# hbaatz/nerf-tex

Measured on AMD Instinct MI355X. Metric: ray-samples/sec (MLP+composite) at 800x800x64, higher is better.
Workload: dtype f32; 1 GPU; carpet 800x800x64: 640000 all-hit rays x 64 samples per GPU (BASELINE configs[1]), ParamNerf n_parameters=[1, 6], seeded glorot weights, inputs resident in HBM, fused PE+MLP+composite; rays_per_gpu=640000, hit_rays_total=640000, samples_per_ray=64

## Files before the change

nerf_tex_amd/csrc/ntx_backend_chain.hip:

```cpp
#include <algorithm>
#include <cstdio>
#include <cstdlib>
#include "ntx_trainer.h"
#include "ntx_train_device.h"
#include "ntx_encode.h"
namespace ntx_train {
enum { PACK_HIDDEN = 0, PACK_LINEAR = 1, PACK_AUX_ROW = 2, PACK_AUX_RGB = 3, PACK_COPY = 4 };
struct PackSeg {
    const float *src; long long sk, sc;
    int mode;
    int K, ncols, nt;
    float *dst; long long first, count;
};
struct PackArgs { const PackSeg *seg; int n_seg; long long total; };
__global__ void pack_kernel(PackArgs a) {
    const long long e = (long long)blockIdx.x * blockDim.x + threadIdx.x;
    if (e >= a.total) return;
    int lo = 0, hi = a.n_seg - 1;
    while (lo < hi) { const int mid = (lo + hi + 1) >> 1; if (a.seg[mid].first <= e) lo = mid; else hi = mid - 1; }
    const PackSeg &p = a.seg[lo];
    const long long o = e - p.first;
    float v = 0.0f;
    if (p.mode == PACK_COPY) v = p.src[o];
    else if (p.mode == PACK_AUX_ROW) {
        const int h = (int)(o >> 7) & 1, V = (int)(o & 127), k = hidden_row(V, h);
        v = k < p.K ? p.src[k * p.sk] : 0.0f;
    } else if (p.mode == PACK_AUX_RGB) {
        const int c = (int)(o >> 7), h = (int)(o >> 6) & 1, V = (int)(o & 63);
        v = p.src[hidden_row(V, h) * 3 + c];
    } else {
        const int c = (int)(o & 3), lane = (int)((o >> 2) & 63);
        const long long rec = o >> 8;
        const int G = p.nt / 4, g = (int)(rec % G), s = (int)(rec / G);
        const int f = lane & 31, kh = lane >> 5;
        const int k = p.mode == PACK_HIDDEN ? hidden_row(s, kh) : 2 * s + kh, col = 32 * (4 * g + c) + f;
        if (k < p.K && col < p.ncols) v = p.src[k * p.sk + col * p.sc];
    }
    p.dst[o] = v;
}

struct EncodeArgs {
    StepRays r;
    float *posO; int ptiles;
    float *dirO; int dtiles;
    float *dists;
};
template <bool IPE>
__global__ __launch_bounds__(64) void encode_kernel(EncodeArgs args) {
    const StepRays &a = args.r;
    const int lane = threadIdx.x, n = lane & 31, h = lane >> 5, blk = blockIdx.x, part = blockIdx.y;
    const long long m = (long long)blk * 32 + n;
    const bool valid = m < a.M();
    const int ray = valid ? (int)(m / a.S) : 0, s = valid ? (int)(m - (long long)ray * a.S) : 0;
// ... 154 lines not shown
            }); });
        }
    }
}

}
namespace {
using namespace ntx_train;
struct ChainBackend : Backend {
    ntx_trainer *t = nullptr;
    int ptiles = 0, dtiles = 0, PS = 0, DS = 0, fwd_variant = 0;
    TLayer trunk[8], feature, c1, c2, rgb, alpha;
    float *wfwd = nullptr, *wdx = nullptr, *aux = nullptr; size_t fwd_floats = 0, dx_floats = 0;
    PackSeg *pack_seg = nullptr; int n_pack = 0; long long pack_total = 0;
    float *posO = nullptr, *dirO = nullptr;
    float *act = nullptr; long long act_stride = 0;
    unsigned int *bits = nullptr; long long bits_stride = 0;
    float *dirrow = nullptr;
    float *gout = nullptr; long long gout_stride = 0;
    DwJob *jobs = nullptr; int n_jobs = 0; long long total_cost = 0;
    std::vector<DwJob> jobs_host; std::vector<int> reduce_job;
    float *dw_partial = nullptr; ReduceBatch reduce{};
    float *G_pos = nullptr, *G_dir = nullptr; int ld_pos = 0, ld_dir = 0;
    float *ray_pg = nullptr;
    float *act_at(int i) const { return act + (size_t)i * act_stride; }
    float *gout_at(int i) const { return gout + (size_t)i * gout_stride; }
    bool samples_on = false;
    static int blocks_of(long long rows) { return (int)((rows + 31) / 32); }
    unsigned chain_grid(long long rows) const { return (unsigned)std::min<long long>(t->cus, (blocks_of(rows) + 3) / 4); }
    unsigned feat_grid(long long rows) const { return (unsigned)std::min<long long>(2 * (long long)t->cus, (blocks_of(rows) + 3) / 4); }
// ... 42 lines not shown
    };
    auto seg = [&](const float *src, long long sk, long long sc, int mode, int K, int ncols, int nt, int stream, int nsteps) {
        PackSeg s{}; s.src = src; s.sk = sk; s.sc = sc; s.mode = mode; s.K = K; s.ncols = ncols; s.nt = nt;
        const int ring = stream == DX ? DX_RING : RING;
        const long long recs = ((long long)nsteps * (nt / 4) + ring - 1) / ring * ring;
        push(s, stream, floats[stream], recs * 256); floats[stream] += (size_t)recs * 256;
    };
    const float *W = t->w;
    auto fwd_hidden = [&](const TLayer &l, int row0, int nt) { seg(W + l.w + (size_t)row0 * l.out, l.out, 1, PACK_HIDDEN, 256, l.out, nt, FWD, 128); };
    auto fwd_linear = [&](const TLayer &l, int K, int nsteps) { seg(W + l.w, l.out, 1, PACK_LINEAR, K, l.out, 8, FWD, nsteps); };
    fwd_linear(trunk[0], Kp, PS);
    for (int i = 1; i < 8; ++i) {
        if (i == 5) { fwd_linear(trunk[5], Kp, PS); fwd_hidden(trunk[5], Kp, 8); }
        else fwd_hidden(trunk[i], 0, 8);
    }
    fwd_hidden(feature, 0, 8);
    fwd_linear(c1, Kd, DS); fwd_hidden(c1, Kd, 8);
    fwd_hidden(c2, 0, 4);
    const size_t n_fwd_segs = segs.size();
    auto dx_hidden = [&](const TLayer &l, int row0, int K, int nsteps) { seg(W + l.w + (size_t)row0 * l.out, 1, l.out, PACK_HIDDEN, K, 256, 8, DX, nsteps); };
    seg(W + rgb.w, 1, 3, PACK_LINEAR, 3, 128, 4, DX, 2);
    dx_hidden(c2, 0, 128, 64);
    dx_hidden(c1, Kd, 256, 128);
    dx_hidden(feature, 0, 256, 128);
    seg(W + alpha.w, 1, 1, PACK_LINEAR, 1, 256, 8, DX, 1);
    for (int i = 7; i >= 1; --i) dx_hidden(trunk[i], i == 5 ? Kp : 0, 256, 128);
    auto tail = [&](size_t of, int stream) { const long long count = (long long)(stream == DX ? DX_RING : RING) * 256; push(segs[of], stream, floats[stream], count); floats[stream] += (size_t)count; };
    tail(0, FWD); tail(n_fwd_segs, DX);
    auto aux_seg = [&](const float *src, int mode, int K, long long count, size_t at) { PackSeg s{}; s.src = src; s.sk = 1; s.mode = mode; s.K = K; push(s, AUX, at, count); };
    for (int i = 0; i < 8; ++i) aux_seg(W + trunk[i].b, PACK_AUX_ROW, 256, 256, AUX_BIAS + (size_t)i * 256);
    aux_seg(W + feature.b, PACK_AUX_ROW, 256, 256, AUX_BIAS + 8 * 256); aux_seg(W + c1.b, PACK_AUX_ROW, 256, 256, AUX_BIAS + 9 * 256);
    aux_seg(W + c2.b, PACK_AUX_ROW, 128, 256, AUX_BIAS + 10 * 256);
    aux_seg(W + alpha.w, PACK_AUX_ROW, 256, 256, AUX_ALPHA_W); aux_seg(W + alpha.b, PACK_COPY, 1, 1, AUX_ALPHA_B);
    aux_seg(W + rgb.w, PACK_AUX_RGB, 128, 384, AUX_RGB_W); aux_seg(W + rgb.b, PACK_COPY, 3, 3, AUX_RGB_B);
    pack_total = first; n_pack = (int)segs.size(); fwd_floats = floats[FWD]; dx_floats = floats[DX];
    t->mem.alloc(&wfwd, fwd_floats); t->mem.alloc(&wdx, dx_floats); t->mem.alloc(&aux, AUX_FLOATS, true);
    float *const base[3] = {wfwd, wdx, aux};
    for (size_t i = 0; i < segs.size(); ++i) segs[i].dst = (float *)((char *)base[base_of[i]] + (uintptr_t)segs[i].dst);
    t->mem.upload(&pack_seg, segs, "segment");
}

void ChainBackend::build_dw_jobs() {
    const int Kp = t->Kp, Kd = t->Kd;
    std::vector<DwJob> &jobs = jobs_host;
    struct RJ { int job; long long at, count, pair; size_t out; };
    std::vector<RJ> rjobs;
    auto new_job = [&]() { DwJob j{}; for (DwWave &w : j.w) w.shape = -1; jobs.push_back(j); return (int)jobs.size() - 1; };
    auto matrix = [&](int j, int K, int N, size_t g_kernel, long long g_bias, long long *at_bias) {
        const long long at = jobs[j].slot_floats;
        jobs[j].slot_floats += (long long)K * N;
        rjobs.push_back(RJ{j, at, (long long)K * N, 0, g_kernel});
        *at_bias = -1;
        if (g_bias >= 0) { *at_bias = jobs[j].slot_floats; jobs[j].slot_floats += 2 * N; rjobs.push_back(RJ{j, *at_bias, N, N, (size_t)g_bias}); }
        return at;
    };
    auto wave = [&](int j, int w, int shape, const float *A, int rtA, int a0, const float *B, int rtB, int b0, long long at, int K, int N, int c_lo, long long at_bias) {
        DwWave &d = jobs[j].w[w];
        d.A = A; d.rtA = rtA; d.a0 = a0; d.B = B; d.rtB = rtB; d.b0 = b0; d.shape = shape; d.out = at; d.ldc = N; d.row0 = a0 * 32; d.rows_valid = K;
        d.col0 = b0 * 32; d.c_lo = c_lo; d.c_hi = c_lo + N; d.bias_out = a0 == 0 ? at_bias : -1;
        const int cost = shape == 0 ? 256 : shape == 1 ? 198 : 68;
        if (cost > jobs[j].cost) jobs[j].cost = cost;
    };
    auto layer_job = [&](const float *X, const float *dY, size_t g_kernel, size_t g_bias) {
        const int j = new_job(); long long ab; const long long at = matrix(j, 256, 256, g_kernel, (long long)g_bias, &ab);
        for (int w = 0; w < 4; ++w) wave(j, w, 0, X, 8, 4 * (w >> 1), dY, 8, 4 * (w & 1), at, 256, 256, 0, ab);
    };
    for (int i = 7; i >= 1; --i) layer_job(act_at(i - 1), gout_at(10 - i), trunk[i].w + (size_t)(i == 5 ? Kp : 0) * 256, trunk[i].b);
    layer_job(act_at(7), gout_at(2), feature.w, feature.b);
    layer_job(act_at(8), gout_at(1), c1.w + (size_t)Kd * 256, c1.b);
    {
        const int j = new_job(); long long ab0, ab5;
        const long long at0 = matrix(j, Kp, 256, trunk[0].w, (long long)trunk[0].b, &ab0), at5 = matrix(j, Kp, 256, trunk[5].w, -1, &ab5);
        for (int w = 0; w < 2; ++w) { wave(j, w, 1, posO, ptiles, 0, gout_at(10), 8, 4 * w, at0, Kp, 256, 0, ab0); wave(j, 2 + w, 1, posO, ptiles, 0, gout_at(5), 8, 4 * w, at5, Kp, 256, 0, ab5); }
    }
    {
        const int j = new_job(); long long abd, ab2;
        const long long atd = matrix(j, Kd, 256, c1.w, -1, &abd), at2 = matrix(j, 256, 128, c2.w, (long long)c2.b, &ab2);
        for (int w = 0; w < 2; ++w) { wave(j, w, 1, dirO, dtiles, 0, gout_at(1), 8, 4 * w, atd, Kd, 256, 0, abd); wave(j, 2 + w, 0, act_at(9), 8, 4 * w, gout_at(0), 4, 0, at2, 256, 128, 0, ab2); }
    }
    {
        const int j = new_job(); long long abr, aba;
        const long long atr = matrix(j, 128, 3, rgb.w, (long long)rgb.b, &abr), ata = matrix(j, 256, 1, alpha.w, (long long)alpha.b, &aba);
        wave(j, 0, 2, act_at(10), 4, 0, t->dhead, 1, 0, atr, 128, 3, 0, abr);
        for (int w = 0; w < 2; ++w) wave(j, 1 + w, 2, act_at(7), 8, 4 * w, t->dhead, 1, 0, ata, 256, 1, 3, aba);
    }
    n_jobs = (int)jobs.size();
    size_t partial_floats = 0;
    for (DwJob &j : jobs) total_cost += j.cost;
    for (DwJob &j : jobs) {
        const long long slots = ((long long)j.cost * t->cus + total_cost - 1) / total_cost + 2;
        j.first_float = (long long)partial_floats; partial_floats += (size_t)(slots * j.slot_floats);
    }
    t->mem.alloc(&dw_partial, partial_floats);
    t->mem.upload(&this->jobs, jobs, "job");
    if (t->mem.rc == NTX_OK && (int)rjobs.size() > MAX_REDUCE_BATCH) t->mem.rc = ntx_set_error(NTX_E_INVALID, "trainer: too many weight gradients for one launch");
    long long rfirst = 0;
    for (size_t i = 0; i < rjobs.size() && t->mem.rc == NTX_OK; ++i) {
        ReduceJob &r = reduce.job[reduce.n++];
        const DwJob &j = jobs[rjobs[i].job];
        r.partial = dw_partial + j.first_float + rjobs[i].at; r.n_split = 0; r.stride = j.slot_floats; r.count = rjobs[i].count; r.pair = rjobs[i].pair;
        r.out = t->grad + rjobs[i].out; r.first = rfirst;
        rfirst += (rjobs[i].count + 255) / 256 * 256;
        reduce_job.push_back(rjobs[i].job);
    }
}

void ChainBackend::launch_pack(hipStream_t st) {
    const PackArgs pa{pack_seg, n_pack, pack_total};
    hipLaunchKernelGGL(pack_kernel, dim3((unsigned)((pack_total + 255) / 256)), dim3(256), 0, st, pa);
}
FwdArgs ChainBackend::fwd_args(long long M) const {
    FwdArgs f{}; f.stream = wfwd; f.stream_bytes = (uint32_t)(fwd_floats * sizeof(float)); f.aux = aux; f.M = M;
    f.ptiles = ptiles; f.dtiles = dtiles; f.pos = posO; f.dir = dirO;
    f.act = act; f.act_stride = act_stride; f.bits = bits; f.bits_stride = bits_stride;
    f.sigma = t->sigma; f.raw_rgb = t->raw_rgb;
    return f;
}
int ChainBackend::forward(const StepRays &r, hipStream_t st) {
    launch_pack(st);
    EncodeArgs e{}; e.r = r; e.posO = posO; e.ptiles = ptiles; e.dirO = dirO; e.dtiles = dtiles; e.dists = t->dists;
    if (t->ipe) hipLaunchKernelGGL(encode_kernel<true>, dim3((unsigned)r.n_blocks(), 2), dim3(64), 0, st, e);
    else hipLaunchKernelGGL(encode_kernel<false>, dim3((unsigned)r.n_blocks(), 2), dim3(64), 0, st, e);
    FwdArgs f = fwd_args(r.M());
    const bool hoist = (t->ipe || r.blur_idx < 0 || r.blur_idx < r.n_geo) && r.S % 32 == 0 && getenv("NERFTEX_TRAIN_NO_DIR_HOIST") == nullptr;
    if (hoist) {
        DirRowArgs dr{}; dr.r = r; dr.Kd = t->Kd; dr.w = t->w + c1.w; dr.bias = t->w + c1.b; dr.rows = dirrow; dr.splice = t->ipe ? r.blur_idx : -1;
        hipLaunchKernelGGL(dirrow_kernel, dim3((unsigned)r.n_rays), dim3(256), 0, st, dr);
    }
    f.dirrow = dirrow; f.n_rays = (int)r.n_rays; f.S = r.S;
    launch_fwd_chain(fwd_variant, hoist, st, chain_grid(r.M()), f);
    return NTX_OK;
}
int ChainBackend::forward_samples(const StepSamples &s, hipStream_t st) {
    if (int rc = takes_samples()) return rc;
    const long long M = s.n_live;
    if (M == 0) return NTX_OK;
    launch_pack(st);
    EncodeSamplesArgs e{}; e.s = s; e.posO = posO; e.ptiles = ptiles; e.dirO = dirO; e.dtiles = dtiles;
    hipLaunchKernelGGL(encode_samples_kernel, dim3((unsigned)blocks_of(M), 2), dim3(64), 0, st, e);
    FwdArgs f = fwd_args(M);
    f.dirrow = dirrow; f.n_rays = (int)s.n_rays; f.S = s.S;
// ... 23 lines not shown
    for (long long g = 0; g < G; ++g) {
        const unsigned long long *c = &h[g * (2 + 3 * n_jobs)];
        fprintf(f, "%lld %llu %llu", g, c[0] - t0, c[1] - t0);
        for (int j = 0; j < n_jobs; ++j) if (c[4 + 3 * j]) fprintf(f, "  j%d cost %d blocks %llu %llu-%llu", j, jobs[j].cost, c[2 + 3 * j], c[3 + 3 * j] - t0, c[4 + 3 * j] - t0);
        fprintf(f, "\n");
    }
    fclose(f);
}
#endif

void ChainBackend::backward_network(long long M, hipStream_t st) {
    DxArgs x{}; x.stream = wdx; x.stream_bytes = (uint32_t)(dx_floats * sizeof(float)); x.M = M; x.dgrad = t->dgrad;
    x.out = gout; x.out_stride = gout_stride; x.bits = bits; x.bits_stride = bits_stride;
    launch_dx_chain(st, chain_grid(M), x);
    if (t->pg_mode != 0 || t->ig_mode != 0) {
        FeatGradArgs p{}; p.dY[0] = gout_at(10); p.W[0] = t->w + trunk[0].w; p.dY[1] = gout_at(5); p.W[1] = t->w + trunk[5].w; p.n_terms = 2;
        p.K = t->Kp; p.ld = ld_pos; p.M = M; p.G = G_pos;
        launch_feat_grad(st, feat_grid(M), ptiles, p);
        FeatGradArgs d{}; d.dY[0] = gout_at(1); d.W[0] = t->w + c1.w; d.n_terms = 1; d.K = t->Kd; d.ld = ld_dir; d.M = M; d.G = G_dir;
        launch_feat_grad(st, feat_grid(M), dtiles, d);
    }
    if (t->takes_weight_gradients()) backward_weights(blocks_of(M), st);
}
int ChainBackend::backward(const StepRays &r, hipStream_t st) {
    backward_network(r.M(), st);
    if (t->pg_mode != 0) {
        const ntx_model_desc &m = t->desc;
        launch_param_fold(st, r, G_pos + 3 * (1 + 2 * m.pos_freq), G_dir + 3 * (1 + 2 * m.dir_freq), ld_pos, ld_dir, ray_pg, t->P, t->param_grad);
    }
    if (t->ig_mode != 0) launch_ray_fold(st, r, G_pos, G_dir, ld_pos, ld_dir, t->dgrad, t->sigma, t->step_noise, t->d_rays_o, t->d_rays_d);
    return NTX_OK;
// ... 26 lines not shown
#endif
    launch_dw(st, (unsigned)G, d);
#ifdef NTX_TRAIN_CLOCKS
    if (d.clocks) dump_dw_clocks(d.clocks, G, jobs_host, st);
#endif
    ReduceBatch rb = reduce;
    std::vector<int> slots(n_jobs);
    long long start = 0;
    for (int j = 0; j < n_jobs; ++j) {
        const long long span = (long long)jobs_host[j].cost * n_blocks;
        slots[j] = (int)(dw_last_g(G, W, start, span) - dw_first_g(G, W, start) + 1);
        start += span;
    }
    for (int i = 0; i < rb.n; ++i) rb.job[i].n_split = slots[reduce_job[i]];
    launch_reduce(st, rb);
}

void ChainBackend::launch_feat_grad(hipStream_t st, unsigned grid, int tiles, const FeatGradArgs &a) {
    if (tiles <= 1) hipLaunchKernelGGL(feat_grad_kernel<1>, dim3(grid), dim3(256), 0, st, a);
    else if (tiles == 2) hipLaunchKernelGGL(feat_grad_kernel<2>, dim3(grid), dim3(256), 0, st, a);
    else hipLaunchKernelGGL(feat_grad_kernel<3>, dim3(grid), dim3(256), 0, st, a);
}

int ChainBackend::enable_gradients(int param_mode, int input_mode) {
    if (param_mode == 0 && input_mode == 0) return NTX_OK;
    if (t->ipe) return ntx_set_error(NTX_E_UNSUPPORTED, "parameter / input gradients of an IPE model on the fused chain: the cone gaussians' derivative is not written");
    if (G_pos) return NTX_OK;
    DeviceMemory &mem = t->mem;
    TRAIN_TRY(hipSetDevice(t->device));
    ld_pos = pad4(t->Kp); ld_dir = pad4(t->Kd);
    mem.alloc(&G_dir, (size_t)t->cap * ld_dir);
    mem.alloc(&ray_pg, (size_t)t->cap_rays * t->P); mem.alloc(&t->param_grad, (size_t)t->cap_rays * t->P);
    mem.alloc(&t->d_rays_o, (size_t)t->cap_rays * 3); mem.alloc(&t->d_rays_d, (size_t)t->cap_rays * 3);
    mem.alloc(&G_pos, (size_t)t->cap * ld_pos);
    return mem.rc;
}

int ChainBackend::activation(int layer, int64_t n_samples_total, float *out_host) {
    const float *src = nullptr; int tiles = 8;
    if (layer >= 0 && layer < 8) src = act_at(layer);
    else if (layer == 8) src = act_at(9);
    else if (layer == 9) { src = act_at(10); tiles = 4; }
    else if (layer == 10) src = t->sigma;
    else if (layer >= 20 && layer < 28) src = gout_at(10 - (layer - 20));
    else if (layer == 28) src = gout_at(1);
    else if (layer == 29) src = gout_at(2);
    else if (layer == 11) src = t->raw_rgb;
    else if (layer == 30) src = t->dgrad;
    else if ((layer == 40 || layer == 41) && G_pos && ((t->pg_mode != 0 && (t->pg_rows > 0 || t->spg_rays > 0)) || (t->ig_mode != 0 && (t->ig_rays > 0 || t->ig_smp_rays > 0)))) src = layer == 40 ? G_pos : G_dir;
    else return ntx_set_error(NTX_E_INVALID, "layer %d (0-7 trunk, 8 / 9 the colour layers, 10 the density, 11 the raw colour; 20-29 the kept gradients, 30 the composite's adjoint; "
                              "40 / 41 the gradient at pos_map / dir_map of a step under ntx_trainer_enable_gradients)", layer);
    TRAIN_TRY(hipSetDevice(t->device));
    TRAIN_TRY(hipDeviceSynchronize());
    if (layer == 40 || layer == 41) {
        const int K = layer == 40 ? t->Kp : t->Kd, ld = layer == 40 ? ld_pos : ld_dir;
        TRAIN_TRY(hipMemcpy2D(out_host, (size_t)K * sizeof(float), src, (size_t)ld * sizeof(float), (size_t)K * sizeof(float), (size_t)n_samples_total, hipMemcpyDeviceToHost));
        return NTX_OK;
    }
    if (layer == 10 || layer == 11 || layer == 30) {
        const size_t width = layer == 10 ? 1 : (layer == 11 ? 3 : 4);
        TRAIN_TRY(hipMemcpy(out_host, src, (size_t)n_samples_total * width * sizeof(float), hipMemcpyDeviceToHost)); return NTX_OK;
    }
    const long long nb = (n_samples_total + 31) / 32;
    std::vector<float> tmp((size_t)nb * tiles * 1024);
    TRAIN_TRY(hipMemcpy(tmp.data(), src, tmp.size() * sizeof(float), hipMemcpyDeviceToHost));
    const int width = tiles * 32;
    for (long long m = 0; m < n_samples_total; ++m)
        for (int row = 0; row < width; ++row) out_host[(size_t)m * width + row] = tmp[o_index(m >> 5, tiles, row, (int)(m & 31))];
// ... 20 lines not shown
    if (Kp > 8 * MAX_PB_GROUPS || Kd > 8 * MAX_PB_GROUPS)
        return ntx_set_error(NTX_E_UNSUPPORTED, "training: pos_map (%d) / dir_map (%d) wider than %d features (the chain holds a block's encoded inputs in registers)", Kp, Kd,
                             8 * MAX_PB_GROUPS);
    dims->desc = *desc; dims->Kp = Kp; dims->Kd = Kd; dims->ipe = ipe; dims->n_weights = ChainBackend().plan_layers(*desc, ipe);
    return NTX_OK;
}

int chain_backend_create(ntx_trainer *t) {
    ChainBackend *c = new ChainBackend();
    t->backend = c; c->t = t;
    c->plan_layers(t->desc, t->ipe);
    DeviceMemory &mem = t->mem;
    const long long NB = t->cap_blocks;
    mem.alloc(&c->posO, (size_t)NB * c->ptiles * 1024, true); mem.alloc(&c->dirO, (size_t)NB * c->dtiles * 1024, true);
    c->act_stride = c->gout_stride = NB * 8 * 1024; c->bits_stride = NB * 256;
    mem.alloc(&c->act, (size_t)c->act_stride * 11); mem.alloc(&c->bits, (size_t)c->bits_stride * 10); mem.alloc(&c->gout, (size_t)c->gout_stride * 11);
    mem.alloc(&c->dirrow, (size_t)t->cap_rays * 256);
    c->build_pack();
    c->build_dw_jobs();
    return mem.rc;
}
}
```

nerf_tex_amd/csrc/ntx_train_device.h:

```cpp
#pragma once

#include "ntx_device.h"

namespace ntx_train {

using ntx::f32x16;
using ntx::f32x4;
using ntx::hidden_row;
using ntx::mfma32;
using ntx::RING;
using ntx::static_for;
typedef float f32x2 __attribute__((ext_vector_type(2)));
typedef int i32x4 __attribute__((ext_vector_type(4)));
typedef unsigned int u32x4 __attribute__((ext_vector_type(4)));

#define TRN_DEV __device__ __forceinline__

TRN_DEV __amdgpu_buffer_rsrc_t make_rsrc(const void *base, long long bytes) {
    const long long b = bytes < 0 ? 0 : (bytes > 0x7ffffff0ll ? 0x7ffffff0ll : bytes);
    return __builtin_amdgcn_make_buffer_rsrc(const_cast<void *>(base), 0, (int)b, 0x00020000);
}

TRN_DEV uint32_t o_lane_bytes(int lane) {
    const int n = lane & 31, h = lane >> 5;
// ... 109 lines not shown
        : "a"(prev[T][R + 0]), "a"(prev[T][R + 1]), "a"(prev[T][R + 2]), "a"(prev[T][R + 3]), "a"(prev[T][R + 4]), "a"(prev[T][R + 5]), "a"(prev[T][R + 6]),
          "a"(prev[T][R + 7]));
}
constexpr int keep_bit(int V) { return 31 - (V & 31); }

template <int NMT>
TRN_DEV void convert_relu_bits(float (&hin)[128], const f32x16 (&prev)[8], u32x4 &bits) {
    static_for<(NMT + 1) / 2>([&](auto W) {
        constexpr int wd = W;
        uint32_t w = 0;
        static_for<(NMT - 2 * wd >= 2 ? 4 : 2)>([&](auto Q) { convert8_relu_bits<32 * wd + 8 * decltype(Q)::value>(hin, prev, w); });
        bits[wd] = w;
    });
}
template <int NMT>
TRN_DEV void convert_linear(float (&hin)[128], const f32x16 (&prev)[8]) {
    static_for<NMT * 16>([&](auto V) { constexpr int v = V; hin[v] = prev[v >> 4][v & 15]; });
}
template <int NMT>
TRN_DEV void convert_mask(float (&hin)[128], const f32x16 (&prev)[8], const u32x4 &bits) {
    static_for<NMT * 16>([&](auto V) {
        constexpr int v = V;
        const float x = prev[v >> 4][v & 15];
        const int keep = __builtin_amdgcn_sbfe((int)bits[v >> 5], keep_bit(v), 1);
        hin[v] = __builtin_bit_cast(float, __builtin_bit_cast(int, x) & keep);
    });
}

constexpr int AUX_BIAS = 0, AUX_ALPHA_W = 11 * 256, AUX_ALPHA_B = AUX_ALPHA_W + 256, AUX_RGB_W = AUX_ALPHA_B + 4, AUX_RGB_B = AUX_RGB_W + 384,
              AUX_FLOATS = AUX_RGB_B + 4;
template <int MT>
TRN_DEV void bias_tile(f32x16 (&acc)[8], const float *aux, int layer, int h) {
    const f32x4 *b = reinterpret_cast<const f32x4 *>(aux + AUX_BIAS + layer * 256 + h * 128) + MT * 4;
    const f32x4 v0 = b[0], v1 = b[1], v2 = b[2], v3 = b[3];
    acc[MT] = f32x16{v0.x, v0.y, v0.z, v0.w, v1.x, v1.y, v1.z, v1.w, v2.x, v2.y, v2.z, v2.w, v3.x, v3.y, v3.z, v3.w};
}

constexpr int MAX_PB_GROUPS = 12;
struct FwdArgs {
    const float *stream; uint32_t stream_bytes;
    const float *aux;
    long long M;
    int ptiles, dtiles;
    const float *pos, *dir;
    float *act; long long act_stride;
    unsigned int *bits; long long bits_stride;
    float *sigma, *raw_rgb;
    const float *dirrow; int n_rays, S;
};

#ifdef NTX_TRAIN_FWD
template <int PSG, int DSG, bool HOIST>
__global__ __launch_bounds__(256) __attribute__((amdgpu_waves_per_eu(1, 1))) void fwd_chain_kernel(FwdArgs a) {
    __shared__ __attribute__((aligned(16))) float aux_lds[AUX_FLOATS];
    __shared__ __attribute__((aligned(16))) float rows_lds[HOIST ? 4 * 256 : 4];
    ntx::load_aux(aux_lds, a.aux, AUX_FLOATS);
    const int lane = threadIdx.x & 63, n = lane & 31, h = lane >> 5;
    const int wave = __builtin_amdgcn_readfirstlane(blockIdx.x * 4 + (threadIdx.x >> 6)), nwaves = gridDim.x * 4;
    const int n_blocks = (int)((a.M + 31) >> 5);
    if (wave >= n_blocks) return;
    WRing ws;
    ws.rsrc = make_rsrc(a.stream, a.stream_bytes);
    ws.voff = (uint32_t)lane * 16u;
    static_for<RING>([&](auto I) { ws.r[I] = wr_load(ws, (uint32_t)decltype(I)::value * 1024u); });
    const uint32_t lane_o = o_lane_bytes(lane), lane_r = (uint32_t)((n >> 3) * 1024 + ((n >> 2) & 1) * 512 + (n & 3) * 4 + h * 16), lane16 = (uint32_t)lane * 16u;
    float pb[12];
    const __amdgpu_buffer_rsrc_t rs_row = make_rsrc(a.dirrow, HOIST ? (long long)a.n_rays * 1024 : 0);
    __amdgpu_buffer_rsrc_t rs_in = make_rsrc(a.pos + (size_t)wave * a.ptiles * 1024, (long long)a.ptiles * 4096);
    auto fetch = [&](auto G) {
        constexpr int g = G;
        static_for<4>([&](auto K) {
            constexpr int k = K;
            constexpr int s = 4 * g + k;
            pb[4 * (g % 3) + k] = __builtin_bit_cast(float, __builtin_amdgcn_raw_buffer_load_b32(rs_in, lane_r, (uint32_t)((s >> 4) * 4096 + (s & 15) * 32), 0));
        });
    };
    fetch(std::integral_constant<int, 0>{}); fetch(std::integral_constant<int, 1>{});
    for (int blk = wave; blk < n_blocks; blk += nwaves) {
        uint32_t opaque_zero = 0;
        asm volatile("" : "+v"(opaque_zero));
        const float *aux = aux_lds + opaque_zero;
        const float *rows_aux = rows_lds + opaque_zero + (HOIST ? (threadIdx.x >> 6) * 256 : 0) - AUX_BIAS - 9 * 256;
        uint32_t sbase = 0;
        f32x16 acc[8];
        float hin[128];
        const long long m = (long long)blk * 32 + n;
        const bool valid = m < a.M;
        if constexpr (HOIST) {
            const uint32_t ray = __builtin_amdgcn_readfirstlane((int)(((uint32_t)blk * 32u) / (uint32_t)a.S));
            const f32x4 x0 = __builtin_bit_cast(f32x4, __builtin_amdgcn_raw_buffer_load_b128(rs_row, lane16, (ray < (uint32_t)a.n_rays ? ray : (uint32_t)a.n_rays - 1u) * 1024u, 0));
            *reinterpret_cast<f32x4 *>(rows_lds + (threadIdx.x >> 6) * 256 + lane * 4) = x0;
            __builtin_amdgcn_wave_barrier();
        }
        __amdgpu_buffer_rsrc_t rs_out = make_rsrc(a.act, 0);
        auto leaves_to = [&](int idx, int tiles) { rs_out = make_rsrc(a.act + (size_t)idx * a.act_stride + (size_t)blk * tiles * 1024, (long long)tiles * 4096); };
        auto leave = [&](auto V) {
            constexpr int v = V;
// ... 1 lines not shown
            __builtin_amdgcn_raw_buffer_store_b32(__builtin_bit_cast(int, hin[v]), rs_out, lane_o, o_value_bytes(v), STORE_NT);
#endif
        };
        auto bits_leave = [&](int idx, const u32x4 &bw) {
#ifndef NTX_X_NOBITS
            const __amdgpu_buffer_rsrc_t rb = make_rsrc(a.bits + (size_t)idx * a.bits_stride + (size_t)blk * 256, 1024);
            __builtin_amdgcn_raw_buffer_store_b128(__builtin_bit_cast(i32x4, bw), rb, lane16, 0, 0);
#endif
        };
        static_for<8>([&](auto T) { bias_tile<decltype(T)::value>(acc, aux, 0, h); });
        seg_mem<PSG>(acc, ws, sbase, pb, fetch);
        float sig_part = 0.0f;
        auto layer = [&](auto LIc) {
            f32x16 (&cur)[8] = acc; f32x16 (&prev)[8] = acc;
            constexpr int LI = decltype(LIc)::value, in_idx = LI - 1;
            constexpr bool relu_in = in_idx != 8;
            u32x4 bw = {0u, 0u, 0u, 0u};
            if constexpr (HOIST && LI == 9) {
                sbase += (uint32_t)DSG * 8192u;
                static_for<RING>([&](auto I) { ws.r[I] = wr_load(ws, sbase + (uint32_t)decltype(I)::value * 1024u); });
            }
            static_for<4>([&](auto W) {
                constexpr int wd = W;
                if constexpr (relu_in) {
                    uint32_t w = 0;
                    static_for<4>([&](auto Q) { convert8_relu_bits<32 * wd + 8 * decltype(Q)::value>(hin, prev, w); });
                    bw[wd] = w;
                } else static_for<32>([&](auto V) { constexpr int v = 32 * wd + decltype(V)::value; hin[v] = prev[v >> 4][v & 15]; });
                const float *bsrc = (HOIST && LI == 9) ? rows_aux : aux;
                if constexpr (LI < 10 || wd < 2) { bias_tile<2 * wd>(cur, bsrc, LI, h); bias_tile<2 * wd + 1>(cur, bsrc, LI, h); }
            });
            if constexpr (relu_in) bits_leave(in_idx < 8 ? in_idx : 8, bw);
            if constexpr (LI == 8) {
                const f32x4 *wa = reinterpret_cast<const f32x4 *>(aux + AUX_ALPHA_W + h * 128);
                static_for<32>([&](auto I) {
                    constexpr int i = I;
                    const f32x4 w = wa[i];
                    sig_part = __builtin_fmaf(hin[4 * i + 0], w.x, sig_part); sig_part = __builtin_fmaf(hin[4 * i + 1], w.y, sig_part);
                    sig_part = __builtin_fmaf(hin[4 * i + 2], w.z, sig_part); sig_part = __builtin_fmaf(hin[4 * i + 3], w.w, sig_part);
                });
            }
            __builtin_amdgcn_sched_barrier(0);
            leaves_to(in_idx, 8);
            if constexpr (LI == 5) seg_mem<PSG>(cur, ws, sbase, pb, fetch);
            if constexpr (LI == 9 && !HOIST) seg_mem<DSG>(cur, ws, sbase, pb, fetch);
            if constexpr (LI == 4) rs_in = make_rsrc(a.pos + (size_t)blk * a.ptiles * 1024, (long long)a.ptiles * 4096);
            if constexpr (LI == 8 && !HOIST) rs_in = make_rsrc(a.dir + (size_t)blk * a.dtiles * 1024, (long long)a.dtiles * 4096);
            if constexpr (LI == 10) {
                const int nb = blk + nwaves < n_blocks ? blk + nwaves : blk;
                rs_in = make_rsrc(a.pos + (size_t)nb * a.ptiles * 1024, (long long)a.ptiles * 4096);
            }
            auto extra = [&](auto S, auto MT) {
                constexpr int s = decltype(S)::value, mt = decltype(MT)::value;
                if constexpr ((LI == 4 || (LI == 8 && !HOIST) || LI == 10) && mt == 2 && (s == 8 || s == 24)) fetch(std::integral_constant<int, (s == 8 ? 0 : 1)>{});
                if constexpr (mt == 5 || (LI == 10 && mt == 3)) leave(S);
            };
            if constexpr (LI == 10) seg_hidden<128, 4, false>(cur, ws, sbase, hin, extra);
            else seg_hidden<128, 8, false>(cur, ws, sbase, hin, extra);
        };
        static_for<10>([&](auto I) { layer(std::integral_constant<int, decltype(I)::value + 1>{}); });
        {
            u32x4 bw = {0u, 0u, 0u, 0u};
            convert_relu_bits<4>(hin, acc, bw);
            bits_leave(9, bw);
            leaves_to(10, 4);
            static_for<64>([&](auto V) { leave(V); });
            float rgb[3];
            static_for<3>([&](auto C) {
                constexpr int c = C;
                const f32x4 *wc = reinterpret_cast<const f32x4 *>(aux + AUX_RGB_W + (c * 2 + h) * 64);
                float p = 0.0f;
                static_for<16>([&](auto I) {
                    constexpr int i = I;
                    const f32x4 w = wc[i];
                    p = __builtin_fmaf(hin[4 * i + 0], w.x, p); p = __builtin_fmaf(hin[4 * i + 1], w.y, p);
                    p = __builtin_fmaf(hin[4 * i + 2], w.z, p); p = __builtin_fmaf(hin[4 * i + 3], w.w, p);
                });
                rgb[c] = p + __shfl_xor(p, 32, 64) + aux[AUX_RGB_B + c];
            });
            const float sigma = sig_part + __shfl_xor(sig_part, 32, 64) + aux[AUX_ALPHA_B];
// ... 5 lines not shown
    }
}

#endif

struct DxArgs {
    const float *stream; uint32_t stream_bytes;
    long long M;
    const float *dgrad;
    float *out; long long out_stride;
    const unsigned int *bits; long long bits_stride;
};

#ifdef NTX_TRAIN_DX
__global__ __launch_bounds__(256) __attribute__((amdgpu_waves_per_eu(1, 1))) void dx_chain_kernel(DxArgs a) {
    const int lane = threadIdx.x & 63, n = lane & 31, h = lane >> 5;
    const int wave = __builtin_amdgcn_readfirstlane(blockIdx.x * 4 + (threadIdx.x >> 6)), nwaves = gridDim.x * 4;
    const int n_blocks = (int)((a.M + 31) >> 5);
    if (wave >= n_blocks) return;
    WRingT<DX_RING> ws;
    ws.rsrc = make_rsrc(a.stream, a.stream_bytes);
    ws.voff = (uint32_t)lane * 16u;
    static_for<DX_RING>([&](auto I) { ws.r[I] = wr_load(ws, (uint32_t)decltype(I)::value * 1024u); });
    const uint32_t lane_o = o_lane_bytes(lane), lane16 = (uint32_t)lane * 16u;
    auto fetch_grad = [&](int blk) {
        const long long m = (long long)blk * 32 + n;
        const f32x4 zero = {0.0f, 0.0f, 0.0f, 0.0f};
        return m < a.M ? *reinterpret_cast<const f32x4 *>(a.dgrad + 4 * m) : zero;
    };
    f32x4 g = fetch_grad(wave);
// ... 14 lines not shown
        u32x4 bw = fetch_bits(9);
        const float gs = h ? 0.0f : g.w;
        {
            const float b[2] = {h ? g.y : g.x, h ? 0.0f : g.z};
            seg_few<2, 4, true>(acc, ws, sbase, b);
        }
        {
            const int nb = blk + nwaves < n_blocks ? blk + nwaves : blk;
            g = fetch_grad(nb);
        }
        convert_mask<4>(hin, acc, bw);
        bw = fetch_bits(8);
        leaves_to(0, 4);
        seg_hidden<64, 8, true>(acc, ws, sbase, hin, [&](auto S, auto MT) { if constexpr (decltype(MT)::value == 5) leave(S); });
        convert_mask<8>(hin, acc, bw);
        leaves_to(1, 8);
        seg_hidden<128, 8, true>(acc, ws, sbase, hin, [&](auto S, auto MT) { if constexpr (decltype(MT)::value == 5) leave(S); });
        convert_linear<8>(hin, acc);
        static_for<8>([&](auto J) {
            constexpr int j = J;
            bw = fetch_bits(7 - j);
            leaves_to(2 + j, 8);
            seg_hidden<128, 8, true>(acc, ws, sbase, hin, [&](auto S, auto MT) { if constexpr (decltype(MT)::value == 5) leave(S); });
            if constexpr (j == 0) {
                const float b[1] = {gs};
                seg_few<1, 8, false>(acc, ws, sbase, b);
            }
            convert_mask<8>(hin, acc, bw);
        });
        leaves_to(10, 8);
        static_for<128>([&](auto V) { leave(V); });
    }
}

#endif

struct DwWave {
    const float *A; int rtA, a0;
    const float *B; int rtB, b0;
    int shape;
    long long out; int ldc;
    int row0, rows_valid, col0, c_lo, c_hi;
    long long bias_out;
};
struct DwJob { DwWave w[4]; int cost; long long slot_floats, first_float; };
// ... 149 lines not shown
```

Measured before the change: 112.6 million ray-samples/s.

## Fold linear feature layer into c1 hidden weights to drop a matmul

```diff
diff --git a/nerf_tex_amd/csrc/ntx_backend_chain.hip b/nerf_tex_amd/csrc/ntx_backend_chain.hip
--- a/nerf_tex_amd/csrc/ntx_backend_chain.hip
+++ b/nerf_tex_amd/csrc/ntx_backend_chain.hip
@@ -37,6 +37,37 @@
         if (k < p.K && col < p.ncols) v = p.src[k * p.sk + col * p.sc];
     }
     p.dst[o] = v;
+}
+
+struct FoldArgs { const float *wf, *bf, *wcf, *bc; float *wfold, *bfold; };
+__global__ __launch_bounds__(256) void fold_kernel(FoldArgs a) {
+    const int i = blockIdx.x, j = threadIdx.x;
+    const float *x = i < 256 ? a.wf + (size_t)i * 256 : a.bf;
+    double acc = i < 256 ? 0.0 : (double)a.bc[j];
+    for (int k = 0; k < 256; ++k) acc = fma((double)x[k], (double)a.wcf[(size_t)k * 256 + j], acc);
+    (i < 256 ? a.wfold + (size_t)i * 256 : a.bfold)[j] = (float)acc;
+}
+struct UnfoldArgs { const float *wf, *bf, *wcf, *dwfold, *dbc; float *g_wf, *g_bf, *g_wcf; };
+__global__ __launch_bounds__(256) void unfold_kernel(UnfoldArgs a) {
+    __shared__ float tile[256][33];
+    const int b = blockIdx.x, t = threadIdx.x;
+    double acc = 0.0;
+    if (b < 256) {
+        for (int i = 0; i < 256; ++i) acc = fma((double)a.wf[(size_t)i * 256 + b], (double)a.dwfold[(size_t)i * 256 + t], acc);
+        a.g_wcf[(size_t)b * 256 + t] = (float)fma((double)a.bf[b], (double)a.dbc[t], acc);
+    } else if (b < 512) {
+        const float *row = a.dwfold + (size_t)(b - 256) * 256;
+        for (int j0 = 0; j0 < 256; j0 += 32) {
+            __syncthreads();
+            for (int r = 0; r < 32; ++r) tile[8 * r + (t >> 5)][t & 31] = a.wcf[(size_t)(8 * r + (t >> 5)) * 256 + j0 + (t & 31)];
+            __syncthreads();
+            for (int j = 0; j < 32; ++j) acc = fma((double)row[j0 + j], (double)tile[t][j], acc);
+        }
+        a.g_wf[(size_t)(b - 256) * 256 + t] = (float)acc;
+    } else {
+        for (int j = 0; j < 256; ++j) acc = fma((double)a.wcf[(size_t)t * 256 + j], (double)a.dbc[j], acc);
+        a.g_bf[t] = (float)acc;
+    }
 }
 
 struct EncodeArgs {
@@ -221,6 +252,7 @@
     float *wfwd = nullptr, *wdx = nullptr, *aux = nullptr; size_t fwd_floats = 0, dx_floats = 0;
     PackSeg *pack_seg = nullptr; int n_pack = 0; long long pack_total = 0;
     float *posO = nullptr, *dirO = nullptr;
+    float *wfold = nullptr, *bfold = nullptr, *dwfold = nullptr;
     float *act = nullptr; long long act_stride = 0;
     unsigned int *bits = nullptr; long long bits_stride = 0;
     float *dirrow = nullptr;
@@ -293,23 +325,22 @@
         if (i == 5) { fwd_linear(trunk[5], Kp, PS); fwd_hidden(trunk[5], Kp, 8); }
         else fwd_hidden(trunk[i], 0, 8);
     }
-    fwd_hidden(feature, 0, 8);
-    fwd_linear(c1, Kd, DS); fwd_hidden(c1, Kd, 8);
+    fwd_linear(c1, Kd, DS);
+    seg(wfold, 256, 1, PACK_HIDDEN, 256, 256, 8, FWD, 128);
     fwd_hidden(c2, 0, 4);
     const size_t n_fwd_segs = segs.size();
     auto dx_hidden = [&](const TLayer &l, int row0, int K, int nsteps) { seg(W + l.w + (size_t)row0 * l.out, 1, l.out, PACK_HIDDEN, K, 256, 8, DX, nsteps); };
     seg(W + rgb.w, 1, 3, PACK_LINEAR, 3, 128, 4, DX, 2);
     dx_hidden(c2, 0, 128, 64);
-    dx_hidden(c1, Kd, 256, 128);
-    dx_hidden(feature, 0, 256, 128);
+    seg(wfold, 1, 256, PACK_HIDDEN, 256, 256, 8, DX, 128);
     seg(W + alpha.w, 1, 1, PACK_LINEAR, 1, 256, 8, DX, 1);
     for (int i = 7; i >= 1; --i) dx_hidden(trunk[i], i == 5 ? Kp : 0, 256, 128);
     auto tail = [&](size_t of, int stream) { const long long count = (long long)(stream == DX ? DX_RING : RING) * 256; push(segs[of], stream, floats[stream], count); floats[stream] += (size_t)count; };
     tail(0, FWD); tail(n_fwd_segs, DX);
     auto aux_seg = [&](const float *src, int mode, int K, long long count, size_t at) { PackSeg s{}; s.src = src; s.sk = 1; s.mode = mode; s.K = K; push(s, AUX, at, count); };
     for (int i = 0; i < 8; ++i) aux_seg(W + trunk[i].b, PACK_AUX_ROW, 256, 256, AUX_BIAS + (size_t)i * 256);
-    aux_seg(W + feature.b, PACK_AUX_ROW, 256, 256, AUX_BIAS + 8 * 256); aux_seg(W + c1.b, PACK_AUX_ROW, 256, 256, AUX_BIAS + 9 * 256);
-    aux_seg(W + c2.b, PACK_AUX_ROW, 128, 256, AUX_BIAS + 10 * 256);
+    aux_seg(bfold, PACK_AUX_ROW, 256, 256, AUX_BIAS + 8 * 256);
+    aux_seg(W + c2.b, PACK_AUX_ROW, 128, 256, AUX_BIAS + 9 * 256);
     aux_seg(W + alpha.w, PACK_AUX_ROW, 256, 256, AUX_ALPHA_W); aux_seg(W + alpha.b, PACK_COPY, 1, 1, AUX_ALPHA_B);
     aux_seg(W + rgb.w, PACK_AUX_RGB, 128, 384, AUX_RGB_W); aux_seg(W + rgb.b, PACK_COPY, 3, 3, AUX_RGB_B);
     pack_total = first; n_pack = (int)segs.size(); fwd_floats = floats[FWD]; dx_floats = floats[DX];
@@ -322,15 +353,15 @@
 void ChainBackend::build_dw_jobs() {
     const int Kp = t->Kp, Kd = t->Kd;
     std::vector<DwJob> &jobs = jobs_host;
-    struct RJ { int job; long long at, count, pair; size_t out; };
+    struct RJ { int job; long long at, count, pair; float *out; };
     std::vector<RJ> rjobs;
     auto new_job = [&]() { DwJob j{}; for (DwWave &w : j.w) w.shape = -1; jobs.push_back(j); return (int)jobs.size() - 1; };
-    auto matrix = [&](int j, int K, int N, size_t g_kernel, long long g_bias, long long *at_bias) {
+    auto matrix = [&](int j, int K, int N, float *g_kernel, long long g_bias, long long *at_bias) {
         const long long at = jobs[j].slot_floats;
         jobs[j].slot_floats += (long long)K * N;
         rjobs.push_back(RJ{j, at, (long long)K * N, 0, g_kernel});
         *at_bias = -1;
-        if (g_bias >= 0) { *at_bias = jobs[j].slot_floats; jobs[j].slot_floats += 2 * N; rjobs.push_back(RJ{j, *at_bias, N, N, (size_t)g_bias}); }
+        if (g_bias >= 0) { *at_bias = jobs[j].slot_floats; jobs[j].slot_floats += 2 * N; rjobs.push_back(RJ{j, *at_bias, N, N, t->grad + g_bias}); }
         return at;
     };
     auto wave = [&](int j, int w, int shape, const float *A, int rtA, int a0, const float *B, int rtB, int b0, long long at, int K, int N, int c_lo, long long at_bias) {
@@ -340,27 +371,26 @@
         const int cost = shape == 0 ? 256 : shape == 1 ? 198 : 68;
         if (cost > jobs[j].cost) jobs[j].cost = cost;
     };
-    auto layer_job = [&](const float *X, const float *dY, size_t g_kernel, size_t g_bias) {
+    auto layer_job = [&](const float *X, const float *dY, float *g_kernel, size_t g_bias) {
         const int j = new_job(); long long ab; const long long at = matrix(j, 256, 256, g_kernel, (long long)g_bias, &ab);
         for (int w = 0; w < 4; ++w) wave(j, w, 0, X, 8, 4 * (w >> 1), dY, 8, 4 * (w & 1), at, 256, 256, 0, ab);
     };
-    for (int i = 7; i >= 1; --i) layer_job(act_at(i - 1), gout_at(10 - i), trunk[i].w + (size_t)(i == 5 ? Kp : 0) * 256, trunk[i].b);
-    layer_job(act_at(7), gout_at(2), feature.w, feature.b);
-    layer_job(act_at(8), gout_at(1), c1.w + (size_t)Kd * 256, c1.b);
+    for (int i = 7; i >= 1; --i) layer_job(act_at(i - 1), gout_at(9 - i), t->grad + trunk[i].w + (size_t)(i == 5 ? Kp : 0) * 256, trunk[i].b);
+    layer_job(act_at(7), gout_at(1), dwfold, c1.b);
     {
         const int j = new_job(); long long ab0, ab5;
-        const long long at0 = matrix(j, Kp, 256, trunk[0].w, (long long)trunk[0].b, &ab0), at5 = matrix(j, Kp, 256, trunk[5].w, -1, &ab5);
-        for (int w = 0; w < 2; ++w) { wave(j, w, 1, posO, ptiles, 0, gout_at(10), 8, 4 * w, at0, Kp, 256, 0, ab0); wave(j, 2 + w, 1, posO, ptiles, 0, gout_at(5), 8, 4 * w, at5, Kp, 256, 0, ab5); }
+        const long long at0 = matrix(j, Kp, 256, t->grad + trunk[0].w, (long long)trunk[0].b, &ab0), at5 = matrix(j, Kp, 256, t->grad + trunk[5].w, -1, &ab5);
+        for (int w = 0; w < 2; ++w) { wave(j, w, 1, posO, ptiles, 0, gout_at(9), 8, 4 * w, at0, Kp, 256, 0, ab0); wave(j, 2 + w, 1, posO, ptiles, 0, gout_at(4), 8, 4 * w, at5, Kp, 256, 0, ab5); }
     }
     {
         const int j = new_job(); long long abd, ab2;
-        const long long atd = matrix(j, Kd, 256, c1.w, -1, &abd), at2 = matrix(j, 256, 128, c2.w, (long long)c2.b, &ab2);
-        for (int w = 0; w < 2; ++w) { wave(j, w, 1, dirO, dtiles, 0, gout_at(1), 8, 4 * w, atd, Kd, 256, 0, abd); wave(j, 2 + w, 0, act_at(9), 8, 4 * w, gout_at(0), 4, 0, at2, 256, 128, 0, ab2); }
+        const long long atd = matrix(j, Kd, 256, t->grad + c1.w, -1, &abd), at2 = matrix(j, 256, 128, t->grad + c2.w, (long long)c2.b, &ab2);
+        for (int w = 0; w < 2; ++w) { wave(j, w, 1, dirO, dtiles, 0, gout_at(1), 8, 4 * w, atd, Kd, 256, 0, abd); wave(j, 2 + w, 0, act_at(8), 8, 4 * w, gout_at(0), 4, 0, at2, 256, 128, 0, ab2); }
     }
     {
         const int j = new_job(); long long abr, aba;
-        const long long atr = matrix(j, 128, 3, rgb.w, (long long)rgb.b, &abr), ata = matrix(j, 256, 1, alpha.w, (long long)alpha.b, &aba);
-        wave(j, 0, 2, act_at(10), 4, 0, t->dhead, 1, 0, atr, 128, 3, 0, abr);
+        const long long atr = matrix(j, 128, 3, t->grad + rgb.w, (long long)rgb.b, &abr), ata = matrix(j, 256, 1, t->grad + alpha.w, (long long)alpha.b, &aba);
+        wave(j, 0, 2, act_at(9), 4, 0, t->dhead, 1, 0, atr, 128, 3, 0, abr);
         for (int w = 0; w < 2; ++w) wave(j, 1 + w, 2, act_at(7), 8, 4 * w, t->dhead, 1, 0, ata, 256, 1, 3, aba);
     }
     n_jobs = (int)jobs.size();
@@ -378,13 +408,16 @@
         ReduceJob &r = reduce.job[reduce.n++];
         const DwJob &j = jobs[rjobs[i].job];
         r.partial = dw_partial + j.first_float + rjobs[i].at; r.n_split = 0; r.stride = j.slot_floats; r.count = rjobs[i].count; r.pair = rjobs[i].pair;
-        r.out = t->grad + rjobs[i].out; r.first = rfirst;
+        r.out = rjobs[i].out; r.first = rfirst;
         rfirst += (rjobs[i].count + 255) / 256 * 256;
         reduce_job.push_back(rjobs[i].job);
     }
 }
 
 void ChainBackend::launch_pack(hipStream_t st) {
+    const float *W = t->w;
+    const FoldArgs fa{W + feature.w, W + feature.b, W + c1.w + (size_t)t->Kd * 256, W + c1.b, wfold, bfold};
+    hipLaunchKernelGGL(fold_kernel, dim3(257), dim3(256), 0, st, fa);
     const PackArgs pa{pack_seg, n_pack, pack_total};
     hipLaunchKernelGGL(pack_kernel, dim3((unsigned)((pack_total + 255) / 256)), dim3(256), 0, st, pa);
 }
@@ -403,7 +436,7 @@
     FwdArgs f = fwd_args(r.M());
     const bool hoist = (t->ipe || r.blur_idx < 0 || r.blur_idx < r.n_geo) && r.S % 32 == 0 && getenv("NERFTEX_TRAIN_NO_DIR_HOIST") == nullptr;
     if (hoist) {
-        DirRowArgs dr{}; dr.r = r; dr.Kd = t->Kd; dr.w = t->w + c1.w; dr.bias = t->w + c1.b; dr.rows = dirrow; dr.splice = t->ipe ? r.blur_idx : -1;
+        DirRowArgs dr{}; dr.r = r; dr.Kd = t->Kd; dr.w = t->w + c1.w; dr.bias = bfold; dr.rows = dirrow; dr.splice = t->ipe ? r.blur_idx : -1;
         hipLaunchKernelGGL(dirrow_kernel, dim3((unsigned)r.n_rays), dim3(256), 0, st, dr);
     }
     f.dirrow = dirrow; f.n_rays = (int)r.n_rays; f.S = r.S;
@@ -457,7 +490,7 @@
     x.out = gout; x.out_stride = gout_stride; x.bits = bits; x.bits_stride = bits_stride;
     launch_dx_chain(st, chain_grid(M), x);
     if (t->pg_mode != 0 || t->ig_mode != 0) {
-        FeatGradArgs p{}; p.dY[0] = gout_at(10); p.W[0] = t->w + trunk[0].w; p.dY[1] = gout_at(5); p.W[1] = t->w + trunk[5].w; p.n_terms = 2;
+        FeatGradArgs p{}; p.dY[0] = gout_at(9); p.W[0] = t->w + trunk[0].w; p.dY[1] = gout_at(4); p.W[1] = t->w + trunk[5].w; p.n_terms = 2;
         p.K = t->Kp; p.ld = ld_pos; p.M = M; p.G = G_pos;
         launch_feat_grad(st, feat_grid(M), ptiles, p);
         FeatGradArgs d{}; d.dY[0] = gout_at(1); d.W[0] = t->w + c1.w; d.n_terms = 1; d.K = t->Kd; d.ld = ld_dir; d.M = M; d.G = G_dir;
@@ -514,6 +547,9 @@
     }
     for (int i = 0; i < rb.n; ++i) rb.job[i].n_split = slots[reduce_job[i]];
     launch_reduce(st, rb);
+    const float *w = t->w; float *g = t->grad;
+    const UnfoldArgs ua{w + feature.w, w + feature.b, w + c1.w + (size_t)t->Kd * 256, dwfold, g + c1.b, g + feature.w, g + feature.b, g + c1.w + (size_t)t->Kd * 256};
+    hipLaunchKernelGGL(unfold_kernel, dim3(513), dim3(256), 0, st, ua);
 }
 
 void ChainBackend::launch_feat_grad(hipStream_t st, unsigned grid, int tiles, const FeatGradArgs &a) {
@@ -539,12 +575,11 @@
 int ChainBackend::activation(int layer, int64_t n_samples_total, float *out_host) {
     const float *src = nullptr; int tiles = 8;
     if (layer >= 0 && layer < 8) src = act_at(layer);
-    else if (layer == 8) src = act_at(9);
-    else if (layer == 9) { src = act_at(10); tiles = 4; }
+    else if (layer == 8) src = act_at(8);
+    else if (layer == 9) { src = act_at(9); tiles = 4; }
     else if (layer == 10) src = t->sigma;
-    else if (layer >= 20 && layer < 28) src = gout_at(10 - (layer - 20));
-    else if (layer == 28) src = gout_at(1);
-    else if (layer == 29) src = gout_at(2);
+    else if (layer >= 20 && layer < 28) src = gout_at(9 - (layer - 20));
+    else if (layer == 28 || layer == 29) src = gout_at(1);
     else if (layer == 11) src = t->raw_rgb;
     else if (layer == 30) src = t->dgrad;
     else if ((layer == 40 || layer == 41) && G_pos && ((t->pg_mode != 0 && (t->pg_rows > 0 || t->spg_rays > 0)) || (t->ig_mode != 0 && (t->ig_rays > 0 || t->ig_smp_rays > 0)))) src = layer == 40 ? G_pos : G_dir;
@@ -552,6 +587,19 @@
                               "40 / 41 the gradient at pos_map / dir_map of a step under ntx_trainer_enable_gradients)", layer);
     TRAIN_TRY(hipSetDevice(t->device));
     TRAIN_TRY(hipDeviceSynchronize());
+    if (layer == 29) {
+        float *G = nullptr;
+        TRAIN_TRY(hipMalloc((void **)&G, (size_t)std::max<int64_t>(n_samples_total, 1) * 256 * sizeof(float)));
+        for (int j0 = 0; j0 < 256; j0 += 96) {
+            FeatGradArgs f{}; f.dY[0] = src; f.W[0] = t->w + c1.w + (size_t)(t->Kd + j0) * 256; f.n_terms = 1; f.K = std::min(96, 256 - j0); f.ld = 256; f.M = n_samples_total; f.G = G + j0;
+            launch_feat_grad(nullptr, feat_grid(n_samples_total), (f.K + 31) / 32, f);
+        }
+        hipError_t e = hipDeviceSynchronize();
+        if (e == hipSuccess) e = hipMemcpy(out_host, G, (size_t)n_samples_total * 256 * sizeof(float), hipMemcpyDeviceToHost);
+        (void)hipFree(G);
+        TRAIN_TRY(e);
+        return NTX_OK;
+    }
     if (layer == 40 || layer == 41) {
         const int K = layer == 40 ? t->Kp : t->Kd, ld = layer == 40 ? ld_pos : ld_dir;
         TRAIN_TRY(hipMemcpy2D(out_host, (size_t)K * sizeof(float), src, (size_t)ld * sizeof(float), (size_t)K * sizeof(float), (size_t)n_samples_total, hipMemcpyDeviceToHost));
@@ -602,7 +650,8 @@
     const long long NB = t->cap_blocks;
     mem.alloc(&c->posO, (size_t)NB * c->ptiles * 1024, true); mem.alloc(&c->dirO, (size_t)NB * c->dtiles * 1024, true);
     c->act_stride = c->gout_stride = NB * 8 * 1024; c->bits_stride = NB * 256;
-    mem.alloc(&c->act, (size_t)c->act_stride * 11); mem.alloc(&c->bits, (size_t)c->bits_stride * 10); mem.alloc(&c->gout, (size_t)c->gout_stride * 11);
+    mem.alloc(&c->act, (size_t)c->act_stride * 10); mem.alloc(&c->bits, (size_t)c->bits_stride * 10); mem.alloc(&c->gout, (size_t)c->gout_stride * 10);
+    mem.alloc(&c->wfold, 256 * 256); mem.alloc(&c->bfold, 256); mem.alloc(&c->dwfold, 256 * 256);
     mem.alloc(&c->dirrow, (size_t)t->cap_rays * 256);
     c->build_pack();
     c->build_dw_jobs();
diff --git a/nerf_tex_amd/csrc/ntx_train_device.h b/nerf_tex_amd/csrc/ntx_train_device.h
--- a/nerf_tex_amd/csrc/ntx_train_device.h
+++ b/nerf_tex_amd/csrc/ntx_train_device.h
@@ -147,10 +147,6 @@
     });
 }
 template <int NMT>
-TRN_DEV void convert_linear(float (&hin)[128], const f32x16 (&prev)[8]) {
-    static_for<NMT * 16>([&](auto V) { constexpr int v = V; hin[v] = prev[v >> 4][v & 15]; });
-}
-template <int NMT>
 TRN_DEV void convert_mask(float (&hin)[128], const f32x16 (&prev)[8], const u32x4 &bits) {
     static_for<NMT * 16>([&](auto V) {
         constexpr int v = V;
@@ -160,7 +156,7 @@
     });
 }
 
-constexpr int AUX_BIAS = 0, AUX_ALPHA_W = 11 * 256, AUX_ALPHA_B = AUX_ALPHA_W + 256, AUX_RGB_W = AUX_ALPHA_B + 4, AUX_RGB_B = AUX_RGB_W + 384,
+constexpr int AUX_BIAS = 0, AUX_ALPHA_W = 10 * 256, AUX_ALPHA_B = AUX_ALPHA_W + 256, AUX_RGB_W = AUX_ALPHA_B + 4, AUX_RGB_B = AUX_RGB_W + 384,
               AUX_FLOATS = AUX_RGB_B + 4;
 template <int MT>
 TRN_DEV void bias_tile(f32x16 (&acc)[8], const float *aux, int layer, int h) {
@@ -185,6 +181,7 @@
 #ifdef NTX_TRAIN_FWD
 template <int PSG, int DSG, bool HOIST>
 __global__ __launch_bounds__(256) __attribute__((amdgpu_waves_per_eu(1, 1))) void fwd_chain_kernel(FwdArgs a) {
+    asm volatile("" ::: "a255");
     __shared__ __attribute__((aligned(16))) float aux_lds[AUX_FLOATS];
     __shared__ __attribute__((aligned(16))) float rows_lds[HOIST ? 4 * 256 : 4];
     ntx::load_aux(aux_lds, a.aux, AUX_FLOATS);
@@ -213,7 +210,7 @@
         uint32_t opaque_zero = 0;
         asm volatile("" : "+v"(opaque_zero));
         const float *aux = aux_lds + opaque_zero;
-        const float *rows_aux = rows_lds + opaque_zero + (HOIST ? (threadIdx.x >> 6) * 256 : 0) - AUX_BIAS - 9 * 256;
+        const float *rows_aux = rows_lds + opaque_zero + (HOIST ? (threadIdx.x >> 6) * 256 : 0) - AUX_BIAS - 8 * 256;
         uint32_t sbase = 0;
         f32x16 acc[8];
         float hin[128];
@@ -245,23 +242,20 @@
         auto layer = [&](auto LIc) {
             f32x16 (&cur)[8] = acc; f32x16 (&prev)[8] = acc;
             constexpr int LI = decltype(LIc)::value, in_idx = LI - 1;
-            constexpr bool relu_in = in_idx != 8;
             u32x4 bw = {0u, 0u, 0u, 0u};
-            if constexpr (HOIST && LI == 9) {
+            if constexpr (HOIST && LI == 8) {
                 sbase += (uint32_t)DSG * 8192u;
                 static_for<RING>([&](auto I) { ws.r[I] = wr_load(ws, sbase + (uint32_t)decltype(I)::value * 1024u); });
             }
             static_for<4>([&](auto W) {
                 constexpr int wd = W;
-                if constexpr (relu_in) {
-                    uint32_t w = 0;
-                    static_for<4>([&](auto Q) { convert8_relu_bits<32 * wd + 8 * decltype(Q)::value>(hin, prev, w); });
-                    bw[wd] = w;
-                } else static_for<32>([&](auto V) { constexpr int v = 32 * wd + decltype(V)::value; hin[v] = prev[v >> 4][v & 15]; });
-                const float *bsrc = (HOIST && LI == 9) ? rows_aux : aux;
-                if constexpr (LI < 10 || wd < 2) { bias_tile<2 * wd>(cur, bsrc, LI, h); bias_tile<2 * wd + 1>(cur, bsrc, LI, h); }
+                uint32_t w = 0;
+                static_for<4>([&](auto Q) { convert8_relu_bits<32 * wd + 8 * decltype(Q)::value>(hin, prev, w); });
+                bw[wd] = w;
+                const float *bsrc = (HOIST && LI == 8) ? rows_aux : aux;
+                if constexpr (LI < 9 || wd < 2) { bias_tile<2 * wd>(cur, bsrc, LI, h); bias_tile<2 * wd + 1>(cur, bsrc, LI, h); }
             });
-            if constexpr (relu_in) bits_leave(in_idx < 8 ? in_idx : 8, bw);
+            bits_leave(in_idx, bw);
             if constexpr (LI == 8) {
                 const f32x4 *wa = reinterpret_cast<const f32x4 *>(aux + AUX_ALPHA_W + h * 128);
                 static_for<32>([&](auto I) {
@@ -274,27 +268,27 @@
             __builtin_amdgcn_sched_barrier(0);
             leaves_to(in_idx, 8);
             if constexpr (LI == 5) seg_mem<PSG>(cur, ws, sbase, pb, fetch);
-            if constexpr (LI == 9 && !HOIST) seg_mem<DSG>(cur, ws, sbase, pb, fetch);
+            if constexpr (LI == 8 && !HOIST) seg_mem<DSG>(cur, ws, sbase, pb, fetch);
             if constexpr (LI == 4) rs_in = make_rsrc(a.pos + (size_t)blk * a.ptiles * 1024, (long long)a.ptiles * 4096);
-            if constexpr (LI == 8 && !HOIST) rs_in = make_rsrc(a.dir + (size_t)blk * a.dtiles * 1024, (long long)a.dtiles * 4096);
-            if constexpr (LI == 10) {
+            if constexpr (LI == 7 && !HOIST) rs_in = make_rsrc(a.dir + (size_t)blk * a.dtiles * 1024, (long long)a.dtiles * 4096);
+            if constexpr (LI == 9) {
                 const int nb = blk + nwaves < n_blocks ? blk + nwaves : blk;
                 rs_in = make_rsrc(a.pos + (size_t)nb * a.ptiles * 1024, (long long)a.ptiles * 4096);
             }
             auto extra = [&](auto S, auto MT) {
                 constexpr int s = decltype(S)::value, mt = decltype(MT)::value;
-                if constexpr ((LI == 4 || (LI == 8 && !HOIST) || LI == 10) && mt == 2 && (s == 8 || s == 24)) fetch(std::integral_constant<int, (s == 8 ? 0 : 1)>{});
-                if constexpr (mt == 5 || (LI == 10 && mt == 3)) leave(S);
+                if constexpr ((LI == 4 || (LI == 7 && !HOIST) || LI == 9) && mt == 2 && (s == 8 || s == 24)) fetch(std::integral_constant<int, (s == 8 ? 0 : 1)>{});
+                if constexpr (mt == 5 || (LI == 9 && mt == 3)) leave(S);
             };
-            if constexpr (LI == 10) seg_hidden<128, 4, false>(cur, ws, sbase, hin, extra);
+            if constexpr (LI == 9) seg_hidden<128, 4, false>(cur, ws, sbase, hin, extra);
             else seg_hidden<128, 8, false>(cur, ws, sbase, hin, extra);
         };
-        static_for<10>([&](auto I) { layer(std::integral_constant<int, decltype(I)::value + 1>{}); });
+        static_for<9>([&](auto I) { layer(std::integral_constant<int, decltype(I)::value + 1>{}); });
         {
             u32x4 bw = {0u, 0u, 0u, 0u};
             convert_relu_bits<4>(hin, acc, bw);
             bits_leave(9, bw);
-            leaves_to(10, 4);
+            leaves_to(9, 4);
             static_for<64>([&](auto V) { leave(V); });
             float rgb[3];
             static_for<3>([&](auto C) {
@@ -330,6 +324,7 @@
 
 #ifdef NTX_TRAIN_DX
 __global__ __launch_bounds__(256) __attribute__((amdgpu_waves_per_eu(1, 1))) void dx_chain_kernel(DxArgs a) {
+    asm volatile("" ::: "a255");
     const int lane = threadIdx.x & 63, n = lane & 31, h = lane >> 5;
     const int wave = __builtin_amdgcn_readfirstlane(blockIdx.x * 4 + (threadIdx.x >> 6)), nwaves = gridDim.x * 4;
     const int n_blocks = (int)((a.M + 31) >> 5);
@@ -374,13 +369,10 @@
         leaves_to(0, 4);
         seg_hidden<64, 8, true>(acc, ws, sbase, hin, [&](auto S, auto MT) { if constexpr (decltype(MT)::value == 5) leave(S); });
         convert_mask<8>(hin, acc, bw);
-        leaves_to(1, 8);
-        seg_hidden<128, 8, true>(acc, ws, sbase, hin, [&](auto S, auto MT) { if constexpr (decltype(MT)::value == 5) leave(S); });
-        convert_linear<8>(hin, acc);
         static_for<8>([&](auto J) {
             constexpr int j = J;
             bw = fetch_bits(7 - j);
-            leaves_to(2 + j, 8);
+            leaves_to(1 + j, 8);
             seg_hidden<128, 8, true>(acc, ws, sbase, hin, [&](auto S, auto MT) { if constexpr (decltype(MT)::value == 5) leave(S); });
             if constexpr (j == 0) {
                 const float b[1] = {gs};
@@ -388,7 +380,7 @@
             }
             convert_mask<8>(hin, acc, bw);
         });
-        leaves_to(10, 8);
+        leaves_to(9, 8);
         static_for<128>([&](auto V) { leave(V); });
     }
 }
```

Result: no change. 112.8 million ray-samples/s, median of 6 (+0.2%).
